# caidao22/pnode

Hardware: AMD Instinct MI355X
Metric: time-steps/sec (fwd+adjoint) (higher is better)
Workload: dtype f32; 1 GPU; C3a: MLP dynamics 3x512 tanh, batch 4096 x state_dim 512 per GPU, rk4 fixed h=0.01, 100 time steps, adjoint on, stages stored in HBM; batch_per_gpu=4096, state_elements_per_gpu=2097152, rejected_attempts=0, launch_mode=graph(auto), graph_revalidate_every=100, linear_param_grads=engine (8 of 8 parameter tensors; fused dW + db MFMA kernel on 4 layers), stage_tapes_retained=True, tunableop=False, parallelism=batch-sharded x1, one RCCL all-reduce of dL/dtheta per backward

## Files before the change

### __graft_entry__.py

```python
import os

os.environ.setdefault("DEBUG_CLR_GRAPH_PACKET_CAPTURE", "0")
import shutil
import subprocess
import sys

ROOT = os.path.dirname(os.path.abspath(__file__))
if ROOT not in sys.path:
    sys.path.insert(0, ROOT)

CSRC = os.path.join(ROOT, "pnode_amd", "csrc")
LIB = os.path.join(ROOT, "pnode_amd", "lib", "libpnode_amd.so")
SOURCES = [os.path.join(CSRC, "pn_kernels.hip"), os.path.join(CSRC, "pn_krylov.hip"), os.path.join(CSRC, "pn_linear.hip"), os.path.join(CSRC, "pn_dense.hip"), os.path.join(CSRC, "pn_tgrad.hip"),
           os.path.join(CSRC, "pn_rows.hip"),
           os.path.join(CSRC, "pn_ts.cpp"),
           os.path.join(CSRC, "pn_spill.cpp"), os.path.join(CSRC, "pn_steploop.cpp")]
HEADERS = [os.path.join(ROOT, "include", "pnode_amd.h"), os.path.join(CSRC, "pn_internal.h"), os.path.join(CSRC, "pn_device.h"),
           os.path.join(CSRC, "pn_adapt.h"), os.path.join(CSRC, "pn_dispatch.h"), os.path.join(CSRC, "pn_launch.h")]


def _source_hash():
    import hashlib
    h = hashlib.sha256()
    h.update(" ".join(_compile_cmd("hipcc", "OUT")).encode())
    for path in SOURCES + HEADERS:
        h.update(os.path.relpath(path, ROOT).encode() + b"\0")
        with open(path, "rb") as fh:
            h.update(fh.read())
    return h.hexdigest()


def _compile_cmd(hipcc, out):
    return [hipcc, "--offload-arch=gfx950", "-O3", "-std=c++17", "-fPIC", "-shared",
            "-I" + os.path.relpath(os.path.join(ROOT, "include"), ROOT), "-I" + os.path.relpath(CSRC, ROOT)] + \
           [os.path.relpath(p, ROOT) for p in SOURCES] + ["-o", out]

# ... 77 lines not shown
```

### include/pnode_amd.h

```cpp
#ifndef PNODE_AMD_H
#define PNODE_AMD_H

#include <stdint.h>

#ifdef __cplusplus
extern "C" {
#endif

#define PN_MAX_STAGES 7
#define PN_MAX_TERMS 8
#define PN_WGRAD_MAX_PAIRS 8
#define PN_WGRAD_EXACT_FP32 1
#define PN_WGRAD_TILE_64 2
#define PN_ABI_VERSION 4

typedef enum { PN_F32 = 0, PN_F64 = 1 } pn_dtype;

const char *pn_last_error(void);
int pn_abi_version(void);

typedef struct {
  int s;
  int order;
  int fsal;
// ... 35 lines not shown
int pn_param_accum(void *stream, int dtype, void *mu, double alpha, int nseg, const void *const *g,
                   const int64_t *offset, const int64_t *len);

int pn_param_accum_multi(void *stream, int dtype, void *mu, int nsrc, const double *alpha, int nseg,
                         const void *const *g, const int64_t *offset, const int64_t *len);

int pn_colsum_accum_multi(void *stream, int dtype, int nsrc, const int64_t *rows, const int64_t *cols, const void *const *g,
                          void *const *mu, const double *alpha, void *work);
int64_t pn_colsum_work_bytes(int nsrc, const int64_t *rows, const int64_t *cols);
int pn_colsum_accum(void *stream, int dtype, int64_t rows, int64_t cols, const void *g, void *mu, double alpha, void *work);

typedef struct {
  const void *g, *x;
  void *pw, *pb;
  double alpha;
  int64_t out_f, in_f;
} pn_wgrad_pair;
int pn_linear_wgrad_supported(int dtype, int64_t rows, int64_t out_f, int64_t in_f);
int64_t pn_linear_wgrad_work_bytes(int dtype, int64_t out_f, int64_t in_f, int64_t *bias_bytes);
int pn_linear_wgrad(void *stream, int dtype, int64_t rows, int64_t out_f, int64_t in_f, const void *g, const void *x, double alpha,
                    void *pw, void *pb);
int pn_linear_wgrad_group(void *stream, int dtype, int64_t rows, int npairs, const pn_wgrad_pair *pairs, int flags);
int pn_linear_wgrad_finish(void *stream, int dtype, int64_t out_f, int64_t in_f, void *pw, void *pb, void *mu_w, void *mu_b);

int pn_dots(void *stream, int dtype, int64_t n, const void *x, int nk, const void *const *y,
            void *work, double *result_dev);
int64_t pn_dots_work_bytes(int64_t n);
int pn_lincomb(void *stream, int dtype, int64_t n, void *out, int nin, const void *const *x, const double *c);
int pn_stream_wait_scalars(void *stream, const double *host_ptr, int count, double *values);

int pn_copy(void *stream, int dtype, int64_t n, void *y, const void *x);
int pn_zero(void *stream, int dtype, int64_t n, void *y);

typedef enum { PN_K_STAGE = 0, PN_K_COMBINE_WRMS, PN_K_ADJ_THETA, PN_K_ADJ_ACCUM,
               PN_K_PARAM_ACCUM, PN_K_COPY, PN_K_DOTS, PN_K_LINCOMB, PN_K_LINEAR_WGRAD, PN_K_COUNT } pn_kernel_id;
int pn_prof_enable(int on);
int pn_prof_is_enabled(void);
int pn_tune_set(const char *spec);
int pn_prof_collect(int count, int64_t *launches, double *usec, double *bytes);
const char *pn_kernel_name(int kernel_id);

typedef struct pn_ts pn_ts;

pn_ts *pn_ts_create(void);
void pn_ts_destroy(pn_ts *ts);
int pn_ts_set_rk_type(pn_ts *ts, const char *rk_type);
// ... 135 lines not shown
```

### pnode_amd/_lib.py

```python
import ctypes
import os

import torch

_HERE = os.path.dirname(os.path.abspath(__file__))
LIB_PATH = os.path.join(_HERE, "lib", "libpnode_amd.so")

PN_MAX_STAGES = 7
PN_MAX_TERMS = 8
PN_F32, PN_F64 = 0, 1
PN_TRAJ_ALL, PN_TRAJ_SOLUTION, PN_TRAJ_BUDGET = 0, 1, 2
KERNEL_IDS = ("pn_rk_stage", "pn_rk_combine_wrms", "pn_adj_theta", "pn_adj_accum", "pn_param_accum", "pn_copy", "pn_dots", "pn_lincomb",
              "pn_linear_wgrad")


class PnError(RuntimeError):
    """A C-ABI entry point returned non-zero (stands where petsc4py.PETSc.Error did)."""


class Tableau(ctypes.Structure):
    _fields_ = [
        ("s", ctypes.c_int), ("order", ctypes.c_int), ("fsal", ctypes.c_int), ("has_embed", ctypes.c_int),
        ("A", (ctypes.c_double * PN_MAX_STAGES) * PN_MAX_STAGES),
        ("b", ctypes.c_double * PN_MAX_STAGES),
# ... 65 lines not shown
    "pn_rk_combine_wrms": (_i, [_vp, _i, _i64, _vp, _vp, _i, _pvp, _pd, _pd, _d, _d, _vp, _vp]),
    "pn_wrms_work_bytes": (_i64, [_i64]),
    "pn_wrms_partials": (_i64, [_i64]),
    "pn_stream_wait_wrms": (_i, [_vp, _vp, _i64, _pd]),
    "pn_pinned_scalar": (_i, [ctypes.POINTER(_vp), ctypes.POINTER(_vp)]),
    "pn_pinned_free": (_i, [_vp]),
    "pn_stream_create": (_i, [_i, ctypes.POINTER(_vp)]),
    "pn_stream_destroy": (_i, [_vp]),
    "pn_pinned_block": (_i, [_i64, ctypes.POINTER(_vp), ctypes.POINTER(_vp)]),
    "pn_stream_wait_scalar": (_i, [_vp, _vp, _pd]),
    "pn_adj_theta": (_i, [_vp, _i, _i64, _vp, _vp, _d, _i, _pvp, _pd]),
    "pn_adj_accum": (_i, [_vp, _i, _i64, _vp, _vp, _i, _pvp, _pd, _vp, _vp, _d]),
    "pn_param_accum": (_i, [_vp, _i, _vp, _d, _i, _pvp, _pi64, _pi64]),
    "pn_param_accum_multi": (_i, [_vp, _i, _vp, _i, _pd, _i, _pvp, _pi64, _pi64]),
    "pn_lincomb": (_i, [_vp, _i, _i64, _vp, _i, _pvp, _pd]),
    "pn_dots": (_i, [_vp, _i, _i64, _vp, _i, _pvp, _vp, _vp]),
    "pn_dots_work_bytes": (_i64, [_i64]),
    "pn_stream_wait_scalars": (_i, [_vp, _vp, _i, _pd]),
    "pn_linear_wgrad_supported": (_i, [_i, _i64, _i64, _i64]),
    "pn_linear_wgrad_work_bytes": (_i64, [_i, _i64, _i64, _pi64]),
    "pn_linear_wgrad": (_i, [_vp, _i, _i64, _i64, _i64, _vp, _vp, _d, _vp, _vp]),
    "pn_linear_wgrad_group": (_i, [_vp, _i, _i64, _i, ctypes.POINTER(WgradPair), _i]),
    "pn_linear_wgrad_finish": (_i, [_vp, _i, _i64, _i64, _vp, _vp, _vp, _vp]),
    "pn_colsum_accum": (_i, [_vp, _i, _i64, _i64, _vp, _vp, _d, _vp]),
    "pn_colsum_accum_multi": (_i, [_vp, _i, _i, _pi64, _pi64, ctypes.POINTER(_vp), ctypes.POINTER(_vp), _pd, _vp]),
    "pn_colsum_work_bytes": (_i64, [_i, _pi64, _pi64]),
    "pn_copy": (_i, [_vp, _i, _i64, _vp, _vp]),
    "pn_zero": (_i, [_vp, _i, _i64, _vp]),
    "pn_prof_enable": (_i, [_i]),
    "pn_prof_is_enabled": (_i, []),
    "pn_tune_set": (_i, [_cp]),
    "pn_prof_collect": (_i, [_i, _pi64, _pd, _pd]),
    "pn_kernel_name": (_cp, [_i]),
    "pn_ts_create": (_vp, []),
    "pn_ts_destroy": (None, [_vp]),
    "pn_ts_set_rk_type": (_i, [_vp, _cp]),
    "pn_ts_get_tableau": (_i, [_vp, ctypes.POINTER(Tableau)]),
    "pn_ts_set_option": (_i, [_vp, _cp, _cp]),
    "pn_ts_is_adaptive": (_i, [_vp]),
    "pn_ts_set_scheme": (_i, [_vp, _i, _i]),
    "pn_ts_get_tolerances": (_i, [_vp, _pd, _pd]),
    "pn_ts_begin": (_i, [_vp, _d, _d, _i, _pd]),
    "pn_ts_attempt": (_i, [_vp, _pd, _pd]),
    "pn_ts_judge": (_i, [_vp, _d, _pi, _pi, _pi]),
    "pn_ts_count_fixed_steps": (_i64, [_vp]),
    "pn_ts_override_next_dt": (_i, [_vp, _d]),
    "pn_ts_steps": (_i64, [_vp]),
# ... 89 lines not shown
```

### pnode_amd/_lineargrad.py

```python
import ctypes
import functools
import warnings
import weakref

import torch
import torch.nn as nn

from ._lib import PnError


class Evaluation(object):
    __slots__ = ("muted", "through", "unfused")

    def __init__(self):
        self.muted = False
        self.unfused = False
        self.through = {}

    def clean(self, out, handled_ids):
        root = getattr(out, "grad_fn", None)
        if root is None:
            return True
        through = self.through
        seen = set()
        stack = [root]
        while stack:
            fn = stack.pop()
            if fn in seen:
                continue
            seen.add(fn)
            if fn in through:
                nxt = through[fn]
                if nxt is not None:
                    stack.append(nxt)
                continue
            var = getattr(fn, "variable", None)
            if var is not None:
                if id(var) in handled_ids:
                    return False
                continue
            for nxt, _ in fn.next_functions:
                if nxt is not None:
                    stack.append(nxt)
        return True


class LinearParamGrads(object):
    def __init__(self, ode):
        self._ode = weakref.ref(ode)
        self.handles = []
        self.slots = {}
        self.shapes = {}
        self.handled = ()
        self.rest = ()
        self.recording = None
        self.n_clean = 0
        self.n_autograd = 0
        self.alpha = None
        self.target = None
        self.checked = False
        self.muted = False
        self.disabled = False
        self.why = None
        self.cot_storage = None
        self.fused = True
        self.partials = {}
        self.pending = []
        self.unit_capture = False
        self.defer = None
        self._fused_ok = {}
        self.side_on = False
        self.side = None
        self.side_priority = True
        self._side_handle = None
        self.inflight = []
        self.events = []

    def install(self, func, params, offsets):
        self.remove()
        if not isinstance(func, nn.Module):
            return False
        index = {id(p): k for k, p in enumerate(params)}
        self.offsets, self.lens = list(offsets), [p.numel() for p in params]
        owners = {}
        for m in func.modules():
            for p in m._parameters.values():
                if p is not None:
                    owners[id(p)] = owners.get(id(p), 0) + 1
        handled = []
        for m in func.modules():
            if type(m) is not nn.Linear:
                continue
            w, b = m.weight, m.bias
            if id(w) not in index or owners.get(id(w), 0) != 1:
                continue
            if b is not None and (id(b) not in index or owners.get(id(b), 0) != 1):
                continue
            kw = index[id(w)]
            kb = index[id(b)] if b is not None else None
            self.slots[id(m)] = (offsets[kw], w.numel(), None if kb is None else offsets[kb], 0 if b is None else b.numel())
            self.shapes[id(m)] = (int(w.shape[0]), int(w.shape[1]))
            handled.append(kw)
            if kb is not None:
                handled.append(kb)
            self.handles.append(m.register_forward_hook(self._forward_hook))
        self.handled = tuple(sorted(handled))
        hs = set(handled)
        self.rest = tuple(k for k in range(len(params)) if k not in hs)
        self.checked = False
        return bool(self.handled)

    def remove_hooks_only(self):
        for h in self.handles:
            try:
                h.remove()
            except Exception:
                pass
        self.handles = []

    def remove(self):
        self.remove_hooks_only()
        self.slots, self.handled, self.rest = {}, (), ()
        self.shapes, self.partials = {}, {}
        self._fused_ok = {}

    def __del__(self):
        self.remove()
        if self._side_handle is not None:
            lib, h = self._side_handle
            self._side_handle = None
            try:
                lib.pn_stream_destroy(h)
            except Exception:
                pass

    @property
    def active(self):
        return bool(self.handled) and not self.disabled

    def begin(self):
        self.recording = Evaluation()

    def end(self, out, handled_params):
        ev, self.recording = self.recording, None
        if ev is None or out is None:
            return True
        try:
            ok = not ev.unfused and ev.clean(out, {id(p) for p in handled_params})
        finally:
            ev.through = None
        if ok:
            self.n_clean += 1
            return True
        ev.muted = True
        self.n_autograd += 1
        return False

    def abort(self):
        ev, self.recording = self.recording, None
        if ev is not None:
            ev.through = None

    def _forward_hook(self, module, inputs, output):
        ev = self.recording
        if ev is None or not isinstance(output, torch.Tensor) or not output.requires_grad or output.grad_fn is None:
            return None
        if id(module) not in self.slots or not inputs or not isinstance(inputs[0], torch.Tensor):
            return None
        x = inputs[0]
        ode0 = self._ode()
        if output.dtype != x.dtype or output.dtype != module.weight.dtype or (ode0 is not None and output.dtype != ode0.tensor_dtype):
            ev.unfused = True
            return None
        if self.unit_capture:
            out_f, in_f = module.weight.shape
            rows = x.numel() // max(in_f, 1)
            ode = self._ode()
            st = self.partials.get(id(module))
            if not (self.fused and st is not None and ode is not None and x.is_cuda and x.dtype == ode.tensor_dtype
                    and ode._ops.linear_wgrad_supported(rows, out_f, in_f)):
                ev.unfused = True
                return None
        output.register_hook(functools.partial(self._grad_hook, module, x.detach(), x._version, ev))
        ev.through[output.grad_fn] = x.grad_fn
        return None

    def _grad_hook(self, module, x, version, ev, g):
        if self.muted or self.disabled or ev.muted:
            return None
        if x._version != version:
# ... 189 lines not shown
```

### pnode_amd/_rk_sweep.py

```python
import contextlib
import ctypes
import warnings

import torch
import torch.nn as nn

from . import _lib, options
from ._lib import PnError, check


class RKSweep(object):
    def _func_with_grad(self, t, y, which="EX"):
        fn, params, names = ((self.funcIM, self._paramsI, self._pnamesI) if which == "IM"
                             else (self.funcEX, self._paramsE, self._pnamesE))
        lin = self._lin if (which == "EX" and self._lin is not None and self._lin.active) else None
        capturing = self.device.type == "cuda" and params and torch.cuda.is_current_stream_capturing()
        seen = tuple(p.detach().requires_grad_(True) for p in params) if capturing else params
        if lin is not None:
            lin.begin()
        out = None
        try:
            if capturing:
                out = torch.func.functional_call(fn, dict(zip(names, seen)), (t, y))
            else:
                out = fn(t, y)
        finally:
            if lin is not None and out is None:
                lin.abort()
        if lin is None or not lin.end(out, [seen[k] for k in lin.handled]):
            return out, seen
        return out, tuple(seen[k] for k in lin.rest)

    def _call_func(self, t, y_flat, tape=None, slot=None):
        if slot is not None and self._sg is not None:
            return self._sg.evaluate(self, slot, t, y_flat, tape)
        y = self._shaped(y_flat)
        if self._tgrad:
            t = self._t_arg(t, tape is not None)
        if tape is not None:
            with torch.enable_grad():
                y = y.detach().requires_grad_(True)
                k, wrt = self._func_with_grad(t, y)
            tape.append((y, k, wrt, t) if self._tgrad else (y, k, wrt))
        else:
            k = self.funcEX(t, y)
        k = self._func_result(k, y_flat)
        self.nfe_forward += 1
        return k

    def _func_result(self, k, y_flat):
        if k.dtype != self.tensor_dtype or k.device != self.device or k.numel() != self.n:
            raise ValueError("func must return a tensor with the state's shape, dtype and device")
        k = k.detach()
        if not k.is_contiguous():
            k = k.contiguous()
        if k.untyped_storage().data_ptr() == y_flat.untyped_storage().data_ptr():
            k = k.clone()
        return k.reshape(-1)

    def _rk_step(self, t, h, u, K0, unew, stage_dest, want_err, tapes=None, t_first=None):
        ops, s, A, b = self._ops, self._s, self._A, self._b
        if self._native:
            return self._rk_step_native(t, h, u, K0, unew, stage_dest, want_err, tapes, t_first)
        plan = self._stage_plan(h)
        K = [None] * s
        for i in range(s):
            if i == 0:
                y = u
            else:
                y = unew if (self._fsal and i == s - 1) else stage_dest(i)
                idx, coef = plan[i]
# ... 191 lines not shown
        lin = self._lin if (which == "EX" and self._lin is not None) else None
        all_params = self._paramsI if which == "IM" else self._paramsE
        keep = True if (self._unit_capture and tape is not None) else None
        tt = None
        if tape is not None:
            y, out, wrt = tape[:3]
            tt = tape[3] if len(tape) > 3 else None
        else:
            self.nfe_backward += 1
        with torch.enable_grad() if tape is None else contextlib.nullcontext():
            if tape is None:
                y = self._shaped(y_flat).detach().requires_grad_(True)
                if self._tgrad and which == "EX":
                    tt = self._t_arg(t, True)
                out, wrt = self._func_with_grad(t if tt is None else tt, y, which)
            cot = self._shaped(w_flat).view(out.shape)
            tgx = (tt,) if (tt is not None and self._tg is not None and which == "EX") else ()
            gt = None
            if tgx:
                self._tg_dot(slot, w_flat, out, alpha)
            hooked = lin is not None and len(wrt) != len(all_params)
            if hooked and not lin.disabled and alpha is not None:
                capturing = self.device.type == "cuda" and torch.cuda.is_current_stream_capturing()
                if not lin.checked and not capturing:
                    ok, worst = lin.self_check(self, out, y, all_params, cot)
                    if not ok:
                        lin.disabled = True
                        lin.why = "its result differed from autograd's at the self-check (relative %.1e)" % worst
                        lin.remove_hooks_only()
                        warnings.warn("pnode_amd: the engine-side accumulation of the nn.Linear layers' parameter sensitivities is "
                                      "switched off for this solver: its result differs from autograd's (relative %.1e) -- a "
                                      "weight or bias of such a layer is also used somewhere else in func.  Results are autograd's; "
                                      "-pn_linear_param_grads 0 silences this." % worst, RuntimeWarning)
                if not lin.disabled:
                    if self._pend_g and self._pend_mixed:
                        self._flush_param_accum()
                    lin.alpha, lin.target = float(alpha), self.adj_p_tensor
                    lin.cot_storage = w_flat.untyped_storage().data_ptr()
                    try:
                        grads = torch.autograd.grad(out, (y,) + wrt + tgx, cot, allow_unused=True, retain_graph=keep)
                    finally:
                        lin.alpha = None
                    if tgx:
                        gt, grads = grads[-1], grads[:-1]
                    grads = (grads[0],) + tuple(lin.expand(grads[1:], len(all_params)))
                    hooked = None
# ... 156 lines not shown
        self._pend_bias_bytes += g2.numel() * g2.element_size()
        if self._accum_mode == "stage" or len(self._pend_bias) >= 32 or self._pend_bias_bytes >= (1 << 30):
            self._flush_bias_accum()

    def _flush_bias_accum(self):
        if self._pend_bias:
            fn = getattr(self._ops, "colsum_accum_multi", None)
            if fn is not None and self._pend_bias[0][0].device.type == "cuda":
                fn(self._pend_bias)
            else:
                for g2, mu_slice, alpha in self._pend_bias:
                    mu_slice.add_(g2.double().sum(0).to(mu_slice.dtype), alpha=alpha)
            self._pend_bias = []
            self._pend_bias_bytes = 0

    @property
    def linear_param_grads(self):
        lin = self._lin
        if lin is None:
            return "autograd (no eligible nn.Linear layer, a theta stepper, or -pn_linear_param_grads 0)"
        if lin.disabled:
            return "autograd (%s)" % lin.why
        note = "; fused dW + db MFMA kernel on %d layers" % len(lin.partials) if lin.partials else ""
        if lin.n_autograd:
            note += "; %d of %d recorded evaluations of func left to autograd (a handled weight or bias is also used outside its layer there, " \
                    "or a layer runs in another precision than its parameters -- autocast)" % (lin.n_autograd, lin.n_autograd + lin.n_clean)
        return "engine (%d of %d parameter tensors%s)" % (len(lin.handled), len(self._paramsE), note)

    def _setup_linear_grads(self):
        opt = str(options.get_all().get("pn_linear_param_grads", "auto"))
        gemm = opt == "gemm"
        on = opt in ("auto", "gemm") or options.truthy(opt, False)
        side = str(options.get_all().get("pn_linear_side_stream", "0"))
        side_on = (side == "same-priority" or options.truthy(side, False)) and self._stepper_kind is None and self.device.type == "cuda"
        exact = options.truthy(options.get_all().get("pn_linear_wgrad_exact", 0), False)
        tile64 = options.truthy(options.get_all().get("pn_linear_wgrad_tile64", 0), False) or side_on
        if hasattr(self._ops, "wgrad_flags"):
            self._ops.wgrad_flags = (_lib.PN_WGRAD_EXACT_FP32 if exact else 0) | (_lib.PN_WGRAD_TILE_64 if tile64 else 0)
        sig = (id(self.funcEX), on, self._stepper_kind in (None, "imex"), tuple(id(p) for p in self._paramsE), gemm, side_on, exact, tile64)
        if sig == self._lin_sig:
            return
        self._lin_sig = sig
        if self._lin is not None:
            self._lin.remove()
            self._lin = None
        if on and sig[2] and self._paramsE:
            from ._lineargrad import LinearParamGrads
            lin = LinearParamGrads(self)
            lin.fused = not gemm
            lin.side_on = side_on
            lin.side_priority = side != "same-priority"
            if lin.install(self.funcEX, self._paramsE, self._poffE if self._stepper_kind == "imex" else self._poff):
                self._lin = lin

    def _flush_param_accum(self):
        self._flush_bias_accum()
        self._pend_mixed = False
        if self._pend_g:
            self._ops.param_accum_multi(self.adj_p_tensor, self._pend_a, self._pend_g, self._poff, self._plen)
            del self._pend_a[:], self._pend_g[:]

    def _begin_adjoint(self, seed):
        if self._traj is None:
            raise RuntimeError("adjoint requested but no trajectory was saved "
                               "(setupTS(enable_adjoint=True) and a differentiable input are required)")
        if self.adj_u_tensor is None:
            self.adj_u_tensor = self._ops.empty(self._npad)
        self.adj_u_flat = self.adj_u_tensor
        self._ops.copy(self.adj_u_flat, seed)
        self._begin_param_adjoint()
        self._traj.begin_reverse()
        self._rev_next = self._nsteps - 1
        if self._lin is not None:
            self._lin.reset()
# ... 241 lines not shown
```

### pnode_amd/_vecops.py

```python
import contextlib
import ctypes
import warnings

import torch
import torch.nn as nn

from . import _lib, options
from ._lib import PnError, check


class HipVecOps(object):

    def __init__(self, device, dtype, n):
        if device.type != "cuda":
            raise RuntimeError(
                "pnode_amd runs on MI355X HIP devices only (got a %s tensor); there is no CPU path" % device.type)
        self.lib = _lib.load()
        self.device, self.dtype, self.n = device, dtype, n
        self.code = _lib.dtype_code(dtype)
        self.work = None
        self.dots_work = None
        self._err_host = self._err_dev = None
        self._pinned_stream = None
        self._seg_cache = {}
# ... 125 lines not shown
        pb = torch.zeros(nb.value // 8, dtype=torch.float64, device=self.device) if bias else None
        return pw, pb

    def linear_wgrad(self, g, x, alpha, pw, pb):
        self.linear_wgrad_group([(g, x, alpha, pw, pb)])

    MAX_WGRAD_PAIRS = _lib.PN_WGRAD_MAX_PAIRS

    wgrad_flags = 0

    def linear_wgrad_group(self, items, stream=None):
        st = self.stream() if stream is None else stream
        for k in range(0, len(items), self.MAX_WGRAD_PAIRS):
            part = items[k:k + self.MAX_WGRAD_PAIRS]
            arr = (_lib.WgradPair * len(part))()
            for q, (g, x, alpha, pw, pb) in zip(arr, part):
                q.g, q.x, q.pw, q.pb = g.data_ptr(), x.data_ptr(), pw.data_ptr(), (None if pb is None else pb.data_ptr())
                q.alpha, q.out_f, q.in_f = alpha, g.shape[1], x.shape[1]
            check(self.lib.pn_linear_wgrad_group(st, self.code, part[0][0].shape[0], len(part), arr, self.wgrad_flags))

    def linear_wgrad_finish(self, out_f, in_f, pw, pb, mu_w, mu_b):
        check(self.lib.pn_linear_wgrad_finish(self.stream(), self.code, out_f, in_f, pw.data_ptr(), None if pb is None else pb.data_ptr(),
                                              mu_w.data_ptr(), None if mu_b is None else mu_b.data_ptr()))

    dense_flags = _lib.PN_DENSE_NONTEMPORAL

    def dense_eval(self, out, u, Ks, coefs):
        m, nk = len(coefs), len(Ks)
        c = (ctypes.c_double * (m * nk))(*[x for row in coefs for x in row])
        check(self.lib.pn_rk_dense_eval(self.stream(), self.code, self.n, u.data_ptr(), nk, (ctypes.c_void_p * nk)(*[k.data_ptr() for k in Ks]),
                                        m, c, out.data_ptr(), out.stride(0), self.dense_flags))

    def dense_adjoint(self, Ds, G, g, coefs, accumulate=False):
        m, nd = g.shape[0], len(Ds)
        c = (ctypes.c_double * max(m * nd, 1))(*[x for row in coefs for x in row])
        check(self.lib.pn_rk_dense_adjoint(self.stream(), self.code, self.n, m, g.data_ptr(), g.stride(0), nd, c,
                                           (ctypes.c_void_p * max(nd, 1))(*[d.data_ptr() for d in Ds]),
                                           None if G is None else G.data_ptr(), 1 if accumulate else 0))

    def _tgrad_work(self):
        w = getattr(self, "_tg_work", None)
        if w is None:
            w = self._tg_work = torch.zeros(self.lib.pn_tgrad_work_bytes(self.n) // 8, dtype=torch.float64, device=self.device)
        return w

    def tgrad_dots(self, acc, xs, ys, coefs, accumulate=True):
# ... 166 lines not shown
```

Before: 931.1 time-steps/s.

## Fuse Linear+Tanh into custom MFMA GEMM kernels with tanh epilogues

After: 610.9 time-steps/s. -34.4%, worse.

```diff
diff --git a/__graft_entry__.py b/__graft_entry__.py
--- a/__graft_entry__.py
+++ b/__graft_entry__.py
@@ -11,7 +11,7 @@
 
 CSRC = os.path.join(ROOT, "pnode_amd", "csrc")
 LIB = os.path.join(ROOT, "pnode_amd", "lib", "libpnode_amd.so")
-SOURCES = [os.path.join(CSRC, "pn_kernels.hip"), os.path.join(CSRC, "pn_krylov.hip"), os.path.join(CSRC, "pn_linear.hip"), os.path.join(CSRC, "pn_dense.hip"), os.path.join(CSRC, "pn_tgrad.hip"),
+SOURCES = [os.path.join(CSRC, "pn_kernels.hip"), os.path.join(CSRC, "pn_krylov.hip"), os.path.join(CSRC, "pn_linear.hip"), os.path.join(CSRC, "pn_linear_act.hip"), os.path.join(CSRC, "pn_dense.hip"), os.path.join(CSRC, "pn_tgrad.hip"),
            os.path.join(CSRC, "pn_rows.hip"),
            os.path.join(CSRC, "pn_ts.cpp"),
            os.path.join(CSRC, "pn_spill.cpp"), os.path.join(CSRC, "pn_steploop.cpp")]
diff --git a/include/pnode_amd.h b/include/pnode_amd.h
--- a/include/pnode_amd.h
+++ b/include/pnode_amd.h
@@ -81,6 +81,12 @@
                     void *pw, void *pb);
 int pn_linear_wgrad_group(void *stream, int dtype, int64_t rows, int npairs, const pn_wgrad_pair *pairs, int flags);
 int pn_linear_wgrad_finish(void *stream, int dtype, int64_t out_f, int64_t in_f, void *pw, void *pb, void *mu_w, void *mu_b);
+
+int pn_linear_act_supported(int dtype, int64_t rows, int64_t out_f, int64_t in_f);
+int pn_linear_tanh_forward(void *stream, int dtype, int64_t rows, int64_t out_f, int64_t in_f, const void *x, const void *w, const void *b,
+                           void *y);
+int pn_linear_tanh_backward(void *stream, int dtype, int64_t rows, int64_t out_f, int64_t in_f, const void *g, const void *w,
+                            const void *y_prev, void *g_in);
 
 int pn_dots(void *stream, int dtype, int64_t n, const void *x, int nk, const void *const *y,
             void *work, double *result_dev);
diff --git a/pnode_amd/_lib.py b/pnode_amd/_lib.py
--- a/pnode_amd/_lib.py
+++ b/pnode_amd/_lib.py
@@ -111,7 +111,10 @@
     "pn_linear_wgrad": (_i, [_vp, _i, _i64, _i64, _i64, _vp, _vp, _d, _vp, _vp]),
     "pn_linear_wgrad_group": (_i, [_vp, _i, _i64, _i, ctypes.POINTER(WgradPair), _i]),
     "pn_linear_wgrad_finish": (_i, [_vp, _i, _i64, _i64, _vp, _vp, _vp, _vp]),
-    "pn_colsum_accum": (_i, [_vp, _i, _i64, _i64, _vp, _vp, _d, _vp]),
+    "pn_linear_act_supported": (_i, [_i, _i64, _i64, _i64]),
+    "pn_linear_tanh_forward": (_i, [_vp, _i, _i64, _i64, _i64, _vp, _vp, _vp, _vp]),
+    "pn_linear_tanh_backward": (_i, [_vp, _i, _i64, _i64, _i64, _vp, _vp, _vp, _vp]),
+    "pn_colsum_accum": (_i,[_vp, _i, _i64, _i64, _vp, _vp, _d, _vp]),
     "pn_colsum_accum_multi": (_i, [_vp, _i, _i, _pi64, _pi64, ctypes.POINTER(_vp), ctypes.POINTER(_vp), _pd, _vp]),
     "pn_colsum_work_bytes": (_i64, [_i, _pi64, _pi64]),
     "pn_copy": (_i, [_vp, _i, _i64, _vp, _vp]),
diff --git a/pnode_amd/_lineargrad.py b/pnode_amd/_lineargrad.py
--- a/pnode_amd/_lineargrad.py
+++ b/pnode_amd/_lineargrad.py
@@ -10,12 +10,13 @@
 
 
 class Evaluation(object):
-    __slots__ = ("muted", "through", "unfused")
+    __slots__ = ("muted", "through", "unfused", "pairs")
 
     def __init__(self):
         self.muted = False
         self.unfused = False
         self.through = {}
+        self.pairs = None
 
     def clean(self, out, handled_ids):
         root = getattr(out, "grad_fn", None)
@@ -46,6 +47,8 @@
 
 
 class LinearParamGrads(object):
+    is_linear_engine = True
+
     def __init__(self, ode):
         self._ode = weakref.ref(ode)
         self.handles = []
@@ -75,6 +78,8 @@
         self._side_handle = None
         self.inflight = []
         self.events = []
+        self.fuse_tanh = "auto"
+        self.pairs = None
 
     def install(self, func, params, offsets):
         self.remove()
@@ -108,6 +113,12 @@
         hs = set(handled)
         self.rest = tuple(k for k in range(len(params)) if k not in hs)
         self.checked = False
+        ode = self._ode()
+        if self.handled and self.fuse_tanh != "0" and ode is not None:
+            from ._lineartanh import Pairs
+            pairs = Pairs(self, ode, self.fuse_tanh)
+            if pairs.find(func, self.slots, [h.id for h in self.handles]):
+                self.pairs = pairs
         return bool(self.handled)
 
     def remove_hooks_only(self):
@@ -119,6 +130,9 @@
         self.handles = []
 
     def remove(self):
+        if self.pairs is not None:
+            self.pairs.close()
+            self.pairs = None
         self.remove_hooks_only()
         self.slots, self.handled, self.rest = {}, (), ()
         self.shapes, self.partials = {}, {}
@@ -140,12 +154,32 @@
 
     def begin(self):
         self.recording = Evaluation()
+        if self.pairs is not None:
+            self.pairs.open()
+
+    def begin_plain(self):
+        return self.pairs is not None and self.pairs.open()
+
+    def end_plain(self):
+        if self.pairs.close():
+            return True
+        self.pairs.switch_off("a Linear layer of a Linear+Tanh pair is used without its Tanh")
+        return False
 
     def end(self, out, handled_params):
         ev, self.recording = self.recording, None
+        if self.pairs is not None:
+            self.pairs.close()
         if ev is None or out is None:
             return True
         try:
+            if ev.pairs is not None:
+                from ._lineartanh import PairsInvalid
+                try:
+                    self.pairs.settle(ev, out)
+                except PairsInvalid as e:
+                    self.pairs.switch_off(str(e))
+                    raise
             ok = not ev.unfused and ev.clean(out, {id(p) for p in handled_params})
         finally:
             ev.through = None
@@ -158,14 +192,19 @@
 
     def abort(self):
         ev, self.recording = self.recording, None
+        if self.pairs is not None:
+            self.pairs.close()
         if ev is not None:
             ev.through = None
+            ev.pairs = None
 
     def _forward_hook(self, module, inputs, output):
         ev = self.recording
         if ev is None or not isinstance(output, torch.Tensor) or not output.requires_grad or output.grad_fn is None:
             return None
         if id(module) not in self.slots or not inputs or not isinstance(inputs[0], torch.Tensor):
+            return None
+        if ev.pairs is not None and self.pairs is not None and self.pairs.owns(ev, output):
             return None
         x = inputs[0]
         ode0 = self._ode()
diff --git a/pnode_amd/_lineartanh.py b/pnode_amd/_lineartanh.py
--- /dev/null
+++ b/pnode_amd/_lineartanh.py
@@ -0,0 +1,319 @@
+import warnings
+import weakref
+
+import torch
+import torch.nn as nn
+import torch.nn.functional as F
+
+
+class PairsInvalid(RuntimeError):
+    """An evaluation used the head of a pair without its Tanh: its result is not func's.  The caller repeats it unfused."""
+
+
+class PairCall(object):
+    __slots__ = ("ev", "prev", "pre_applied", "node", "done_node", "tanh")
+
+    def __init__(self, ev, tanh):
+        self.ev, self.tanh = ev, tanh
+        self.prev = None
+        self.pre_applied = False
+        self.node = self.done_node = None
+
+
+class _EvalState(object):
+    __slots__ = ("calls", "owned", "pending", "done")
+
+    def __init__(self):
+        self.calls, self.owned, self.pending, self.done = [], {}, {}, {}
+
+
+class _Done(torch.autograd.Function):
+
+    @staticmethod
+    def forward(ctx, y):
+        return y.view_as(y)
+
+    @staticmethod
+    def backward(ctx, g):
+        return g
+
+
+class _Linear(torch.autograd.Function):
+    @staticmethod
+    def forward(ctx, x, W, b, pairs, module, call):
+        ops = pairs.ops()
+        if call.tanh:
+            y = torch.empty((x.shape[0], W.shape[0]), dtype=x.dtype, device=x.device)
+            ops.linear_tanh_forward(x, W, b, y)
+        else:
+            y = F.linear(x, W, b)
+        ctx.save_for_backward(x, W, y if call.tanh else None)
+        ctx.pairs, ctx.module, ctx.call, ctx.xver, ctx.has_bias = pairs, module, call, x._version, b is not None
+        return y
+
+    @staticmethod
+    def backward(ctx, gy):
+        x, W, y = ctx.saved_tensors
+        pairs, call = ctx.pairs, ctx.call
+        g = gy.contiguous()
+        if call.tanh and not call.pre_applied:
+            g = torch.ops.aten.tanh_backward(g, y)
+        lin = pairs.lin()
+        if lin is not None:
+            lin._grad_hook(ctx.module, x.detach(), ctx.xver, call.ev, g)
+        gx = gW = gb = None
+        if ctx.needs_input_grad[0]:
+            prev = call.prev
+            if prev is not None and prev.pre_applied:
+                if g.data_ptr() % 16 == 0:
+                    gx = torch.empty_like(x)
+                    pairs.ops().linear_tanh_backward(g, W, x, gx)
+                else:
+                    gx = torch.ops.aten.tanh_backward(g.mm(W), x)
+            else:
+                gx = g.mm(W)
+        if ctx.needs_input_grad[1]:
+            gW = g.t().mm(x)
+        if ctx.has_bias and ctx.needs_input_grad[2]:
+            gb = g.sum(0)
+        return gx, gW, gb, None, None, None
+
+
+def _foreign_hooks(m, own):
+    for name in ("_forward_pre_hooks", "_backward_hooks", "_backward_pre_hooks", "_forward_hooks_with_kwargs", "_forward_pre_hooks_with_kwargs"):
+        if len(getattr(m, name, None) or ()):
+            return True
+    return any(k not in own and not getattr(getattr(h, "__self__", None), "is_linear_engine", False) for k, h in m._forward_hooks.items())
+
+
+class Pairs(object):
+    def __init__(self, lin, ode, mode):
+        self.lin, self._ode = weakref.ref(lin), weakref.ref(ode)
+        self.force = mode == "1"
+        self.heads = {}
+        self.tanhs = {}
+        self.tails = {}
+        self.off = None
+        self.checked = False
+        self.is_open = False
+        self.n_fused = 0
+        self._plain = {}
+        self._ok = {}
+        self._own = ()
+
+    def ops(self):
+        return self._ode()._ops
+
+    def find(self, func, slots, own_hook_ids):
+        self._own = frozenset(own_hook_ids)
+        count = {}
+        for parent in func.modules():
+            for child in parent._modules.values():
+                if child is not None:
+                    count[id(child)] = count.get(id(child), 0) + 1
+        ok_mod = lambda m: count.get(id(m), 0) == 1 and not _foreign_hooks(m, self._own)
+        for seq in func.modules():
+            if not isinstance(seq, nn.Sequential):
+                continue
+            kids = list(seq._modules.values())
+            for k in range(len(kids) - 1):
+                a, t = kids[k], kids[k + 1]
+                if type(a) is nn.Linear and type(t) is nn.Tanh and id(a) in slots and ok_mod(a) and ok_mod(t):
+                    self.heads[id(a)] = (a, t)
+                    self.tanhs[id(t)] = a
+                    nxt = kids[k + 2] if k + 2 < len(kids) else None
+                    if type(nxt) is nn.Linear and id(nxt) in slots and ok_mod(nxt) and not (k + 3 < len(kids) and type(kids[k + 3]) is nn.Tanh):
+                        self.tails[id(nxt)] = nxt
+        for mid in list(self.tails):
+            if mid in self.heads:
+                del self.tails[mid]
+        return bool(self.heads)
+
+    def modules(self):
+        return [a for a, _ in self.heads.values()] + list(self.tanhs_modules()) + list(self.tails.values())
+
+    def tanhs_modules(self):
+        return [t for _, t in self.heads.values()]
+
+    def open(self):
+        ode = self._ode()
+        if self.off is not None or self.is_open or ode is None or ode._sg is not None or getattr(ode, "_unit_capture", False):
+            return False
+        for m in self.modules():
+            if "forward" in m.__dict__ or _foreign_hooks(m, self._own):
+                return False
+        for a, t in self.heads.values():
+            a.__dict__["forward"] = _Bound(self, a, self._linear_forward)
+            t.__dict__["forward"] = _Bound(self, t, self._tanh_forward)
+        for a in self.tails.values():
+            a.__dict__["forward"] = _Bound(self, a, self._linear_forward)
+        self.is_open = True
+        self._plain = {}
+        return True
+
+    def close(self):
+        if not self.is_open:
+            return True
+        self.is_open = False
+        for m in self.modules():
+            if isinstance(m.__dict__.get("forward"), _Bound):
+                del m.__dict__["forward"]
+        left, self._plain = self._plain, {}
+        return not left
+
+    def switch_off(self, why):
+        if self.off is None:
+            self.off = why
+            warnings.warn("pnode_amd: the fused Linear+Tanh kernels (-pn_linear_fuse_tanh) are switched off for this solver: %s.  "
+                          "func runs on its modules' own forwards; -pn_linear_fuse_tanh 0 silences this." % why, RuntimeWarning)
+
+    def _usable(self, m, x):
+        ode = self._ode()
+        W, b = m.weight, m.bias
+        if not (isinstance(x, torch.Tensor) and x.is_cuda and x.dim() == 2) or torch.is_autocast_enabled():
+            return False, "its input is not a 2-D device tensor outside autocast"
+        fp32 = x.dtype == torch.float32 and W.dtype == torch.float32 and (b is None or b.dtype == torch.float32) and ode.tensor_dtype == torch.float32
+        key = (x.shape[0], W.shape[0], W.shape[1])
+        ok = self._ok.get(key)
+        if ok is None:
+            ok = self._ok[key] = bool(ode._ops.linear_act_supported(*key))
+        if not (fp32 and ok and x.shape[1] == W.shape[1]):
+            return False, "dtype %s or shape %s is outside pn_linear_act_supported" % (x.dtype, key)
+        if not (x.is_contiguous() and W.is_contiguous() and x.data_ptr() % 16 == 0 and W.data_ptr() % 16 == 0
+                and (b is None or (b.is_contiguous() and b.data_ptr() % 16 == 0))):
+            return False, "an operand is not contiguous or not 16-byte aligned"
+        return True, None
+
+    def _linear_forward(self, m, x):
+        head = id(m) in self.heads
+        ok, why = self._usable(m, x)
+        if not ok:
+            if self.force and head and why.startswith("dtype"):
+                raise RuntimeError("pnode_amd: -pn_linear_fuse_tanh 1: the Linear+Tanh pair %r is refused: %s" % (m, why))
+            return nn.Linear.forward(m, x)
+        W, b = m.weight, m.bias
+        lin = self.lin()
+        ev = lin.recording if lin is not None else None
+        if not torch.is_grad_enabled() or not (x.requires_grad or W.requires_grad or (b is not None and b.requires_grad)):
+            if not head:
+                return nn.Linear.forward(m, x)
+            y = torch.empty((x.shape[0], W.shape[0]), dtype=x.dtype, device=x.device)
+            self.ops().linear_tanh_forward(x.detach(), W.detach(), None if b is None else b.detach(), y)
+            self._plain[id(m)] = y
+            self.n_fused += 1
+            return y
+        if ev is None:
+            return nn.Linear.forward(m, x)
+        st = ev.pairs
+        if st is None:
+            st = ev.pairs = _EvalState()
+        call = PairCall(ev, head)
+        fed = st.done.get(id(x))
+        if fed is not None and fed[1] is x:
+            call.prev = fed[0]
+        y = _Linear.apply(x, W, b, self, m, call)
+        call.node = y.grad_fn
+        ev.through[y.grad_fn] = x.grad_fn
+        st.calls.append(call)
+        st.owned[id(y)] = y
+        if head:
+            st.pending[id(y)] = (call, m)
+            self.n_fused += 1
+        return y
+
+    def _tanh_forward(self, t, x):
+        a = self.tanhs[id(t)]
+        y = self._plain.get(id(a))
+        if y is not None and y is x:
+            del self._plain[id(a)]
+            return x
+        lin = self.lin()
+        ev = lin.recording if lin is not None else None
+        st = ev.pairs if ev is not None else None
+        if st is not None and st.owned.get(id(x)) is x:
+            hit = st.pending.get(id(x))
+            if hit is not None and hit[1] is a:
+                del st.pending[id(x)]
+                z = _Done.apply(x)
+                hit[0].done_node = z.grad_fn
+                st.done[id(z)] = (hit[0], z)
+                return z
+        return nn.Tanh.forward(t, x)
+
+    def owns(self, ev, output):
+        st = ev.pairs
+        return st is not None and st.owned.get(id(output)) is output
+
+    def settle(self, ev, out):
+        st, ev.pairs = ev.pairs, None
+        if st is None:
+            return
+        try:
+            root = getattr(out, "grad_fn", None)
+            indeg, seen = {}, set()
+            if root is not None:
+                seen.add(root)
+                stack = [root]
+                while stack:
+                    fn = stack.pop()
+                    for nxt, _ in fn.next_functions:
+                        if nxt is None:
+                            continue
+                        indeg[nxt] = indeg.get(nxt, 0) + 1
+                        if nxt not in seen:
+                            seen.add(nxt)
+                            stack.append(nxt)
+            bad = bool(st.pending)
+            for c in st.calls:
+                if c.tanh and c.node in seen and (c.done_node is None or indeg.get(c.node, 0) != 1):
+                    bad = True
+            if bad:
+                raise PairsInvalid("a Linear layer of a Linear+Tanh pair is used without its Tanh")
+            for c in st.calls:
+                p = c.prev
+                if p is not None and c.node in seen and indeg.get(p.node, 0) == 1 and indeg.get(p.done_node, 0) == 1:
+                    p.pre_applied = True
+        finally:
+            for c in st.calls:
+                c.node = c.done_node = None
+            st.calls, st.owned, st.pending, st.done = [], {}, {}, {}
+
+    def check(self, ode, t, y, out, cot, params):
+        self.checked = True
+        lin = self.lin()
+        saved = lin.muted
+        lin.muted = True
+        try:
+            fused = torch.autograd.grad(out, (y,) + tuple(params), cot, allow_unused=True, retain_graph=True)
+            with torch.enable_grad():
+                y2 = y.detach().requires_grad_(True)
+                out2 = ode.funcEX(t, y2)
+            plain = torch.autograd.grad(out2, (y2,) + tuple(params), cot, allow_unused=True)
+        finally:
+            lin.muted = saved
+        worst = 0.0
+        for a, b in [(out.detach(), out2.detach())] + list(zip(fused, plain)):
+            if a is None and b is None:
+                continue
+            if a is None or b is None:
+                return False, float("inf")
+            scale = float(b.abs().max())
+            err = float((a - b).abs().max())
+            worst = max(worst, err / scale if scale > 0 else err)
+        return worst <= 1e-4, worst
+
+    def describe(self):
+        if self.off is not None:
+            return "; Linear+Tanh pairs unfused (%s)" % self.off
+        return "; %d Linear+Tanh pairs on pn_linear_tanh_forward / _backward%s" % (
+            len(self.heads), "" if self.n_fused else " (none used yet: shapes, dtype or launch mode outside the kernels')")
+
+
+class _Bound(object):
+    __slots__ = ("pairs", "module", "fn")
+
+    def __init__(self, pairs, module, fn):
+        self.pairs, self.module, self.fn = pairs, weakref.ref(module), fn
+
+    def __call__(self, x):
+        return self.fn(self.module(), x)
diff --git a/pnode_amd/_rk_sweep.py b/pnode_amd/_rk_sweep.py
--- a/pnode_amd/_rk_sweep.py
+++ b/pnode_amd/_rk_sweep.py
@@ -7,6 +7,7 @@
 
 from . import _lib, options
 from ._lib import PnError, check
+from ._lineartanh import PairsInvalid as _PairsInvalid
 
 
 class RKSweep(object):
@@ -16,20 +17,26 @@
         lin = self._lin if (which == "EX" and self._lin is not None and self._lin.active) else None
         capturing = self.device.type == "cuda" and params and torch.cuda.is_current_stream_capturing()
         seen = tuple(p.detach().requires_grad_(True) for p in params) if capturing else params
-        if lin is not None:
-            lin.begin()
-        out = None
-        try:
-            if capturing:
-                out = torch.func.functional_call(fn, dict(zip(names, seen)), (t, y))
-            else:
-                out = fn(t, y)
-        finally:
-            if lin is not None and out is None:
-                lin.abort()
-        if lin is None or not lin.end(out, [seen[k] for k in lin.handled]):
-            return out, seen
-        return out, tuple(seen[k] for k in lin.rest)
+        for attempt in (0, 1):
+            if lin is not None:
+                lin.begin()
+            out = None
+            try:
+                if capturing:
+                    out = torch.func.functional_call(fn, dict(zip(names, seen)), (t, y))
+                else:
+                    out = fn(t, y)
+            finally:
+                if lin is not None and out is None:
+                    lin.abort()
+            try:
+                if lin is None or not lin.end(out, [seen[k] for k in lin.handled]):
+                    return out, seen
+            except _PairsInvalid:
+                if attempt:
+                    raise
+                continue
+            return out, tuple(seen[k] for k in lin.rest)
 
     def _call_func(self, t, y_flat, tape=None, slot=None):
         if slot is not None and self._sg is not None:
@@ -43,10 +50,22 @@
                 k, wrt = self._func_with_grad(t, y)
             tape.append((y, k, wrt, t) if self._tgrad else (y, k, wrt))
         else:
-            k = self.funcEX(t, y)
+            k = self._func_plain(t, y)
         k = self._func_result(k, y_flat)
         self.nfe_forward += 1
         return k
+
+    def _func_plain(self, t, y):
+        lin = self._lin
+        if lin is None or not lin.active or torch.is_grad_enabled() or not lin.begin_plain():
+            return self.funcEX(t, y)
+        ok = False
+        try:
+            k = self.funcEX(t, y)
+            ok = True
+        finally:
+            ok = lin.end_plain() and ok
+        return k if ok else self.funcEX(t, y)
 
     def _func_result(self, k, y_flat):
         if k.dtype != self.tensor_dtype or k.device != self.device or k.numel() != self.n:
@@ -284,6 +303,11 @@
             hooked = lin is not None and len(wrt) != len(all_params)
             if hooked and not lin.disabled and alpha is not None:
                 capturing = self.device.type == "cuda" and torch.cuda.is_current_stream_capturing()
+                if lin.pairs is not None and not lin.pairs.checked and lin.pairs.off is None and lin.pairs.n_fused and not capturing:
+                    ok, worst = lin.pairs.check(self, t if tt is None else tt, y, out, cot, [all_params[k] for k in lin.handled])
+                    if not ok:
+                        lin.pairs.switch_off("their result differed from plain autograd of the unfused modules at the self-check "
+                                             "(relative %.1e)" % worst)
                 if not lin.checked and not capturing:
                     ok, worst = lin.self_check(self, out, y, all_params, cot)
                     if not ok:
@@ -486,6 +510,8 @@
         if lin.disabled:
             return "autograd (%s)" % lin.why
         note = "; fused dW + db MFMA kernel on %d layers" % len(lin.partials) if lin.partials else ""
+        if lin.pairs is not None:
+            note += lin.pairs.describe()
         if lin.n_autograd:
             note += "; %d of %d recorded evaluations of func left to autograd (a handled weight or bias is also used outside its layer there, " \
                     "or a layer runs in another precision than its parameters -- autocast)" % (lin.n_autograd, lin.n_autograd + lin.n_clean)
@@ -501,7 +527,11 @@
         tile64 = options.truthy(options.get_all().get("pn_linear_wgrad_tile64", 0), False) or side_on
         if hasattr(self._ops, "wgrad_flags"):
             self._ops.wgrad_flags = (_lib.PN_WGRAD_EXACT_FP32 if exact else 0) | (_lib.PN_WGRAD_TILE_64 if tile64 else 0)
-        sig = (id(self.funcEX), on, self._stepper_kind in (None, "imex"), tuple(id(p) for p in self._paramsE), gemm, side_on, exact, tile64)
+        fuse = str(options.get_all().get("pn_linear_fuse_tanh", "auto")).lower()
+        fuse = "auto" if fuse == "auto" else ("1" if options.truthy(fuse, False) else "0")
+        if self._stepper_kind is not None or self.device.type != "cuda":
+            fuse = "0"
+        sig = (id(self.funcEX), on, self._stepper_kind in (None, "imex"), tuple(id(p) for p in self._paramsE), gemm, side_on, exact, tile64, fuse)
         if sig == self._lin_sig:
             return
         self._lin_sig = sig
@@ -514,6 +544,7 @@
             lin.fused = not gemm
             lin.side_on = side_on
             lin.side_priority = side != "same-priority"
+            lin.fuse_tanh = fuse
             if lin.install(self.funcEX, self._paramsE, self._poffE if self._stepper_kind == "imex" else self._poff):
                 self._lin = lin
 
diff --git a/pnode_amd/_vecops.py b/pnode_amd/_vecops.py
--- a/pnode_amd/_vecops.py
+++ b/pnode_amd/_vecops.py
@@ -171,6 +171,17 @@
     def linear_wgrad_finish(self, out_f, in_f, pw, pb, mu_w, mu_b):
         check(self.lib.pn_linear_wgrad_finish(self.stream(), self.code, out_f, in_f, pw.data_ptr(), None if pb is None else pb.data_ptr(),
                                               mu_w.data_ptr(), None if mu_b is None else mu_b.data_ptr()))
+
+    def linear_act_supported(self, rows, out_f, in_f):
+        return bool(self.lib.pn_linear_act_supported(self.code, rows, out_f, in_f))
+
+    def linear_tanh_forward(self, x, w, b, y):
+        check(self.lib.pn_linear_tanh_forward(self.stream(), self.code, x.shape[0], w.shape[0], w.shape[1], x.data_ptr(), w.data_ptr(),
+                                              None if b is None else b.data_ptr(), y.data_ptr()))
+
+    def linear_tanh_backward(self, g, w, y_prev, g_in):
+        check(self.lib.pn_linear_tanh_backward(self.stream(), self.code, g.shape[0], w.shape[0], w.shape[1], g.data_ptr(), w.data_ptr(),
+                                               y_prev.data_ptr(), g_in.data_ptr()))
 
     dense_flags = _lib.PN_DENSE_NONTEMPORAL
 
diff --git a/pnode_amd/csrc/pn_linear_act.hip b/pnode_amd/csrc/pn_linear_act.hip
--- /dev/null
+++ b/pnode_amd/csrc/pn_linear_act.hip
@@ -0,0 +1,226 @@
+#include <hip/hip_runtime.h>
+
+#include <cstdint>
+
+#include "pn_launch.h"
+#include "pnode_amd.h"
+
+namespace {
+
+typedef float f32x16 __attribute__((ext_vector_type(16)));
+typedef float f32x4 __attribute__((ext_vector_type(4)));
+typedef short s16x4 __attribute__((ext_vector_type(4)));
+typedef short s16x8 __attribute__((ext_vector_type(8)));
+typedef unsigned u32x2 __attribute__((ext_vector_type(2)));
+
+constexpr int kThreads = 512, BM = 64, BN = 128, BK = 32;
+constexpr int TN = BN / 64;
+constexpr int PA = BM * 64;
+constexpr int PB = BN * 64;
+constexpr int BUF = 3 * (PA + PB);
+
+__device__ __forceinline__ void split4(const f32x4 v, u32x2 &hi, u32x2 &mid, u32x2 &lo) {
+  unsigned a[4], r1[4], r2[4];
+#pragma unroll
+  for (int e = 0; e < 4; ++e) {
+    a[e] = __float_as_uint(v[e]);
+    const float f1 = v[e] - __uint_as_float(a[e] & 0xFFFF0000u);
+    r1[e] = __float_as_uint(f1);
+    r2[e] = __float_as_uint(f1 - __uint_as_float(r1[e] & 0xFFFF0000u));
+  }
+  hi = u32x2{__builtin_amdgcn_perm(a[1], a[0], 0x07060302u), __builtin_amdgcn_perm(a[3], a[2], 0x07060302u)};
+  mid = u32x2{__builtin_amdgcn_perm(r1[1], r1[0], 0x07060302u), __builtin_amdgcn_perm(r1[3], r1[2], 0x07060302u)};
+  lo = u32x2{__builtin_amdgcn_perm(r2[1], r2[0], 0x07060302u), __builtin_amdgcn_perm(r2[3], r2[2], 0x07060302u)};
+}
+
+__device__ __forceinline__ void six(f32x16 &c, const s16x8 ah, const s16x8 am, const s16x8 al, const s16x8 bh, const s16x8 bm, const s16x8 bl) {
+  c = __builtin_amdgcn_mfma_f32_32x32x16_bf16(ah, bl, c, 0, 0, 0);
+  c = __builtin_amdgcn_mfma_f32_32x32x16_bf16(al, bh, c, 0, 0, 0);
+  c = __builtin_amdgcn_mfma_f32_32x32x16_bf16(am, bm, c, 0, 0, 0);
+  c = __builtin_amdgcn_mfma_f32_32x32x16_bf16(ah, bm, c, 0, 0, 0);
+  c = __builtin_amdgcn_mfma_f32_32x32x16_bf16(am, bh, c, 0, 0, 0);
+  c = __builtin_amdgcn_mfma_f32_32x32x16_bf16(ah, bh, c, 0, 0, 0);
+}
+
+template <bool BACKWARD>
+__device__ __forceinline__ void linear_act_body(const float *__restrict__ A, const float *__restrict__ B, const float *__restrict__ E,
+                                                float *__restrict__ OUT, int N, int K) {
+  __shared__ __attribute__((aligned(16))) char smem[2 * BUF];
+  const int ntn = N / BN;
+  const int tm = blockIdx.x / ntn, tn = blockIdx.x % ntn;
+  const int t = threadIdx.x, lane = t & 63, w = t >> 6;
+  const int kh = w >> 2, wm = w & 1, wn = (w >> 1) & 1;
+  const int nslab = K / BK;
+  f32x4 av, bv[2];
+  f32x16 acc[TN];
+#pragma unroll
+  for (int j = 0; j < TN; ++j)
+#pragma unroll
+    for (int e = 0; e < 16; ++e) acc[j][e] = 0.f;
+  auto swz = [](int r, int c16) { return c16 ^ ((r >> 2) & 3); };
+  auto swzt = [](int k, int c) { return c ^ (((k >> 1) & 1) << 5); };
+
+  auto gload = [&](int slab) {
+    av = *reinterpret_cast<const f32x4 *>(A + (size_t)(tm * BM + (t >> 3)) * K + slab * BK + (t & 7) * 4);
+#pragma unroll
+    for (int v = 0; v < 2; ++v) {
+      const int idx = t + kThreads * v;
+      if constexpr (BACKWARD)
+        bv[v] = *reinterpret_cast<const f32x4 *>(B + (size_t)(slab * BK + (idx >> 5)) * N + tn * BN + (idx & 31) * 4);
+      else
+        bv[v] = *reinterpret_cast<const f32x4 *>(B + (size_t)(tn * BN + (idx >> 3)) * K + slab * BK + (idx & 7) * 4);
+    }
+  };
+  auto lstore = [&](int buf) {
+    char *b = smem + buf * BUF;
+    u32x2 hi, mid, lo;
+    {
+      const int r = t >> 3, kq = t & 7;
+      const int off = r * 64 + swz(r, kq >> 1) * 16 + (kq & 1) * 8;
+      split4(av, hi, mid, lo);
+      *reinterpret_cast<u32x2 *>(b + off) = hi;
+      *reinterpret_cast<u32x2 *>(b + PA + off) = mid;
+      *reinterpret_cast<u32x2 *>(b + 2 * PA + off) = lo;
+    }
+    char *bb = b + 3 * PA;
+#pragma unroll
+    for (int v = 0; v < 2; ++v) {
+      const int idx = t + kThreads * v;
+      split4(bv[v], hi, mid, lo);
+      if constexpr (BACKWARD) {
+        const int k = idx >> 5, c5 = idx & 31, sub = c5 >> 4, lc = c5 & 15;
+        char *p = bb + sub * (3 * PB / 2) + k * 128 + swzt(k, lc * 4) * 2;
+        *reinterpret_cast<u32x2 *>(p) = hi;
+        *reinterpret_cast<u32x2 *>(p + PB / 2) = mid;
+        *reinterpret_cast<u32x2 *>(p + PB) = lo;
+      } else {
+        const int r = idx >> 3, kq = idx & 7;
+        const int off = r * 64 + swz(r, kq >> 1) * 16 + (kq & 1) * 8;
+        *reinterpret_cast<u32x2 *>(bb + off) = hi;
+        *reinterpret_cast<u32x2 *>(bb + PB + off) = mid;
+        *reinterpret_cast<u32x2 *>(bb + 2 * PB + off) = lo;
+      }
+    }
+  };
+  auto frag = [&](const char *part, int row0) -> s16x8 {
+    const int r = row0 + (lane & 31), c16 = kh * 2 + (lane >> 5);
+    return *reinterpret_cast<const s16x8 *>(part + r * 64 + swz(r, c16) * 16);
+  };
+  const int g4 = lane >> 4, q4 = (lane & 15) >> 2, p4 = lane & 3;
+  auto fragt = [&](const char *part, int col0) -> s16x8 {
+    s16x4 r[2];
+#pragma unroll
+    for (int u = 0; u < 2; ++u) {
+      const int k = kh * 16 + 8 * (g4 >> 1) + 4 * u + q4;
+      const int c = col0 + (g4 & 1) * 16 + 4 * p4;
+      r[u] = __builtin_amdgcn_ds_read_tr16_b64_v4i16((__attribute__((address_space(3))) s16x4 *)(part + k * 128 + swzt(k, c) * 2));
+    }
+    const s16x8 f = {r[0][0], r[0][1], r[0][2], r[0][3], r[1][0], r[1][1], r[1][2], r[1][3]};
+    return f;
+  };
+  auto compute = [&](int buf) {
+    const char *b = smem + buf * BUF, *bb = b + 3 * PA;
+    const s16x8 ah = frag(b, wm * 32), am = frag(b + PA, wm * 32), al = frag(b + 2 * PA, wm * 32);
+#pragma unroll
+    for (int j = 0; j < TN; ++j) {
+      s16x8 bh, bm, bl;
+      if constexpr (BACKWARD) {
+        const char *s = bb + wn * (3 * PB / 2);
+        bh = fragt(s, j * 32), bm = fragt(s + PB / 2, j * 32), bl = fragt(s + PB, j * 32);
+      } else {
+        const int row0 = (wn * TN + j) * 32;
+        bh = frag(bb, row0), bm = frag(bb + PB, row0), bl = frag(bb + 2 * PB, row0);
+      }
+      six(acc[j], ah, am, al, bh, bm, bl);
+    }
+  };
+
+  gload(0);
+  lstore(0);
+  if (nslab > 1) gload(1);
+  __syncthreads();
+  for (int s = 0; s < nslab; ++s) {
+    compute(s & 1);
+    if (s + 1 < nslab) lstore((s + 1) & 1);
+    if (s + 2 < nslab) gload(s + 2);
+    __syncthreads();
+  }
+  float(*red)[64] = reinterpret_cast<float(*)[64]>(smem);
+  static_assert(sizeof(smem) >= (size_t)4 * TN * 16 * 64 * 4, "staging of the second K half");
+  if (kh == 1) {
+#pragma unroll
+    for (int j = 0; j < TN; ++j)
+#pragma unroll
+      for (int e = 0; e < 16; ++e) red[((w & 3) * TN + j) * 16 + e][lane] = acc[j][e];
+  }
+  __syncthreads();
+  if (kh == 0) {
+#pragma unroll
+    for (int j = 0; j < TN; ++j) {
+      const int col = tn * BN + (wn * TN + j) * 32 + (lane & 31);
+      float bj = 0.f;
+      if constexpr (!BACKWARD) bj = E ? E[col] : 0.f;
+#pragma unroll
+      for (int e = 0; e < 16; ++e) {
+        const int row = tm * BM + wm * 32 + (e & 3) + 8 * (e >> 2) + 4 * (lane >> 5);
+        const float c = acc[j][e] + red[((w & 3) * TN + j) * 16 + e][lane];
+        float o;
+        if constexpr (BACKWARD) {
+#pragma clang fp contract(off)
+          const float y = E[(size_t)row * N + col];
+          const float y2 = y * y;
+          const float f = 1.f - y2;
+          o = c * f;
+        } else {
+          o = tanhf(c + bj);
+        }
+        OUT[(size_t)row * N + col] = o;
+      }
+    }
+  }
+}
+
+}
+
+__global__ __launch_bounds__(kThreads) void pn_linear_tanh_fwd_kernel(const float *__restrict__ X, const float *__restrict__ W,
+                                                                      const float *__restrict__ bias, float *__restrict__ Y, int out_f, int in_f) {
+  linear_act_body<false>(X, W, bias, Y, out_f, in_f);
+}
+__global__ __launch_bounds__(kThreads) void pn_linear_tanh_bwd_kernel(const float *__restrict__ G, const float *__restrict__ W,
+                                                                      const float *__restrict__ Yprev, float *__restrict__ Gin, int out_f, int in_f) {
+  linear_act_body<true>(G, W, Yprev, Gin, in_f, out_f);
+}
+
+extern "C" {
+
+int pn_linear_act_supported(int dtype, int64_t rows, int64_t out_f, int64_t in_f) {
+  if (dtype != PN_F32) return 0;
+  return (rows > 0 && rows % BM == 0 && rows < (int64_t)1 << 24 && out_f > 0 && out_f % BN == 0 && in_f > 0 && in_f % BN == 0 &&
+          out_f <= 1 << 16 && in_f <= 1 << 16 && (rows / BM) * (out_f / BN) < (int64_t)1 << 30 && (rows / BM) * (in_f / BN) < (int64_t)1 << 30)
+             ? 1
+             : 0;
+}
+
+int pn_linear_tanh_forward(void *stream, int dtype, int64_t rows, int64_t out_f, int64_t in_f, const void *x, const void *w, const void *b,
+                           void *y) {
+  if (!pn_linear_act_supported(dtype, rows, out_f, in_f))
+    return pn::fail("pn_linear_tanh_forward: unsupported dtype or shape (see pn_linear_act_supported)");
+  if (x == nullptr || w == nullptr || y == nullptr) return pn::fail("pn_linear_tanh_forward: null operand");
+  if (!pn::aligned16(x, w, b, y)) return pn::fail("pn_linear_tanh_forward: operands must be 16-byte aligned");
+  const dim3 grid((unsigned)((rows / BM) * (out_f / BN)));
+  return pn::launch("pn_linear_tanh_forward", pn_linear_tanh_fwd_kernel, grid, dim3(kThreads), (hipStream_t)stream, (const float *)x,
+                    (const float *)w, (const float *)b, (float *)y, (int)out_f, (int)in_f);
+}
+
+int pn_linear_tanh_backward(void *stream, int dtype, int64_t rows, int64_t out_f, int64_t in_f, const void *g, const void *w,
+                            const void *y_prev, void *g_in) {
+  if (!pn_linear_act_supported(dtype, rows, out_f, in_f))
+    return pn::fail("pn_linear_tanh_backward: unsupported dtype or shape (see pn_linear_act_supported)");
+  if (g == nullptr || w == nullptr || y_prev == nullptr || g_in == nullptr) return pn::fail("pn_linear_tanh_backward: null operand");
+  if (!pn::aligned16(g, w, y_prev, g_in)) return pn::fail("pn_linear_tanh_backward: operands must be 16-byte aligned");
+  const dim3 grid((unsigned)((rows / BM) * (in_f / BN)));
+  return pn::launch("pn_linear_tanh_backward", pn_linear_tanh_bwd_kernel, grid, dim3(kThreads), (hipStream_t)stream, (const float *)g,
+                    (const float *)w, (const float *)y_prev, (float *)g_in, (int)out_f, (int)in_f);
+}
+
+}
```
